# mikeoliphant/NeuralAudio

Measured on AMD Instinct MI355X. Metric: concurrent 48 kHz real-time streams + Msamples/s/GPU, NAM WaveNet Standard, higher is better.
Workload: dtype f32 (f16x3-split MFMA, f32 accumulate)

## Files before the change

neuralaudio_amd/csrc/wavenet_spec_impl.h:

```cpp
#pragma once

#include <algorithm>
#include <atomic>
#include <cstddef>
#include <cstdlib>

#include <hip/hip_runtime.h>

#include "device_once.h"
#include <cstring>
#include <type_traits>
#include <vector>

#include "tuning.h"
#include "wavenet_split_dev.h"

namespace na
{
	namespace spk
	{
		using namespace sp;

#ifndef NA_SPK_NT_DIL
#define NA_SPK_NT_DIL 256
#endif
#ifndef NA_SPK_NT_LD
#define NA_SPK_NT_LD 0
#endif
#ifndef NA_SPK_NT_ST
#define NA_SPK_NT_ST 0
#endif
#ifndef NA_SPK_DELAY
#define NA_SPK_DELAY 0
#endif
#ifndef NA_SPK_AUX2
#define NA_SPK_AUX2 0
#endif
		typedef __attribute__((address_space(3))) char* LdsPtr;
		__device__ __forceinline__ u32x4 LdsRead16(unsigned addr) { return *reinterpret_cast<__attribute__((address_space(3))) const u32x4*>((LdsPtr)(size_t)addr); }
		__device__ __forceinline__ u32x2 LdsRead8(unsigned addr) { return *reinterpret_cast<__attribute__((address_space(3))) const u32x2*>((LdsPtr)(size_t)addr); }
		__device__ __forceinline__ void LdsWrite16(unsigned addr, u32x4 v) { *reinterpret_cast<__attribute__((address_space(3))) u32x4*>((LdsPtr)(size_t)addr) = v; }

		template <bool COH>
		__device__ __forceinline__ float LoadIn(const float* p)
		{
			if constexpr (COH) return __builtin_bit_cast(float, __hip_atomic_load(reinterpret_cast<const unsigned*>(p), __ATOMIC_RELAXED, __HIP_MEMORY_SCOPE_SYSTEM));
			else return *p;
		}
		template <bool COH>
		__device__ __forceinline__ void StoreOut(float* p, float v)
		{
			if constexpr (COH) __hip_atomic_store(reinterpret_cast<unsigned*>(p), __builtin_bit_cast(unsigned, v), __ATOMIC_RELAXED, __HIP_MEMORY_SCOPE_SYSTEM);
			else *p = v;
		}

		struct ArchA1Base
		{
			static constexpr int K(int, int) { return 3; }
			static constexpr int HEADK = 1;
			static constexpr bool LEAKY = false;
			static constexpr int T = 2, CHUNK = 10;
			static constexpr bool COARSE = false;
			static constexpr bool GUARDHIST = false;
			static constexpr bool FOLD = false;
			static constexpr int SKEW = 0;
			static constexpr bool COMPACT = true;
#ifndef NA_A1_NT_DIL
#define NA_A1_NT_DIL 128
#endif
			static constexpr int NT_DIL = NA_A1_NT_DIL;
		};
#ifndef NA_SPK_SKEW
#define NA_SPK_SKEW 0
#endif
		struct ArchStd : ArchA1Base
		{
			static constexpr int SKEW = NA_SPK_SKEW;
			static constexpr bool FOLD = true;
			static constexpr int NA = 2;
			static constexpr int CH[2] = { 16, 8 };
			static constexpr int NLA[2] = { 10, 10 };
			static constexpr int DIL[2][16] = { { 1, 2, 4, 8, 16, 32, 64, 128, 256, 512 }, { 1, 2, 4, 8, 16, 32, 64, 128, 256, 512 } };
		};
		struct ArchLite : ArchA1Base
		{
			static constexpr int NA = 2;
			static constexpr int CH[2] = { 16, 8 };
			static constexpr int NLA[2] = { 7, 13 };
			static constexpr int DIL[2][16] = { { 1, 2, 4, 8, 16, 32, 64 }, { 128, 256, 512, 1, 2, 4, 8, 16, 32, 64, 128, 256, 512 } };
		};
		struct ArchLite16 : ArchA1Base
		{
			static constexpr int NA = 2;
			static constexpr int CH[2] = { 16, 16 };
			static constexpr int NLA[2] = { 7, 13 };
			static constexpr int DIL[2][16] = { { 1, 2, 4, 8, 16, 32, 64 }, { 128, 256, 512, 1, 2, 4, 8, 16, 32, 64, 128, 256, 512 } };
		};

		struct ArchLite16T1 : ArchLite16 { static constexpr int T = 1; };

		struct ArchA2Base
		{
			static constexpr int NA = 1;
			static constexpr int NLA[2] = { 23, 0 };
			static constexpr int DIL[2][32] = { { 1, 3, 7, 17, 41, 101, 239, 1, 3, 7, 17, 41, 101, 239, 1, 13, 1, 3, 7, 17, 41, 101, 239 }, { 0 } };
			static constexpr int K(int, int l) { return (l == 14 || l == 15) ? 15 : 6; }
			static constexpr int HEADK = 16;
			static constexpr bool LEAKY = true;
			static constexpr int CHUNK = 16;
			static constexpr bool COARSE = true;
			static constexpr bool GUARDHIST = true;
			static constexpr bool FOLD = false;
			static constexpr int SKEW = 0;
			static constexpr bool COMPACT = false;
			static constexpr int NT_DIL = 100;
		};
		struct ArchA2Full : ArchA2Base { static constexpr int CH[2] = { 8, 0 }; static constexpr int T = 2; };
		struct ArchA2Lite : ArchA2Base { static constexpr int CH[2] = { 4, 0 }; static constexpr int T = 4; };

		struct FamStd { typedef ArchStd A0; typedef ArchStd A1; static constexpr int N = 1; };
		struct FamLite { typedef ArchLite A0; typedef ArchLite A1; static constexpr int N = 1; };
		struct FamLitePacked { typedef ArchLite A0; typedef ArchLite16 A1; static constexpr int N = 2; };
		struct FamA2 { typedef ArchA2Full A0; typedef ArchA2Lite A1; static constexpr int N = 2; };
		struct FamLite16T1 { typedef ArchLite16T1 A0; typedef ArchLite16T1 A1; static constexpr int N = 1; };

		enum TapClass { TAP_LDS = 0, TAP_HIST = 1, TAP_BOTH = 2 };

		template <class A>
		struct Tab
		{
			static constexpr int NA = A::NA;
			static constexpr int TotalLayers() { int n = 0; for (int a = 0; a < NA; a++) n += A::NLA[a]; return n; }
			static constexpr int NL = TotalLayers();
			static constexpr int NSTAGES = NL + NA + 1;
			static constexpr int ArrOf(int L) { int a = 0; while (L >= A::NLA[a]) { L -= A::NLA[a]; a++; } return a; }
			static constexpr int InArr(int L) { int a = 0; while (L >= A::NLA[a]) { L -= A::NLA[a]; a++; } return L; }
			static constexpr int Dil(int L) { return A::DIL[ArrOf(L)][InArr(L)]; }
			static constexpr int GPof(int a) { return A::CH[a] / 4; }
			static constexpr bool FirstOfArr(int L) { return InArr(L) == 0; }
			static constexpr bool LastOfArr(int L) { return InArr(L) == A::NLA[ArrOf(L)] - 1; }
			static constexpr int KS(int L) { return A::K(ArrOf(L), InArr(L)); }
			static constexpr bool Fold(int L) { return A::FOLD && KS(L) == 3 && GPof(ArrOf(L)) >= 2; }
			static constexpr int HEADK = A::HEADK;
			static constexpr int NRINGS = NL + (HEADK > 1 ? 1 : 0);
			static constexpr bool ExactRing(int L) { return L < NL && !FirstOfArr(L) && Dil(L) >= FRAMES && (KS(L) - 1) * Dil(L) >= 2 * FRAMES && ((KS(L) - 1) * Dil(L)) % 16 == 0; }
			static constexpr int HistFrames(int L) { return L < NL ? ((KS(L) - 1) * Dil(L) + 15) / 16 * 16 : (HEADK - 1 + 15) / 16 * 16; }
			static constexpr bool CompactRing(int L) { return A::COMPACT && L < NL && KS(L) > 1 && HistFrames(L) <= WN_COMPACT_MAX_HISTORY; }
			static constexpr int RingFrames(int L)
			{
				if (ExactRing(L)) return (KS(L) - 1) * Dil(L);
				if (CompactRing(L)) return 3 * HistFrames(L);
				return HistFrames(L) + FRAMES;
			}
			static constexpr int RingKeep(int L) { return ExactRing(L) ? RingFrames(L) : (CompactRing(L) ? HistFrames(L) : RingFrames(L) - FRAMES); }
			static constexpr int RingG(int L) { return GPof(L < NL ? ArrOf(L) : NA - 1); }
			static constexpr int RingOff(int L)
			{
				int o = WN_HEADER_F4;
				for (int l = 0; l < L; l++) o += RingFrames(l) * RingG(l);
				return o;
			}
			static constexpr int StateF4 = (RingOff(NRINGS) + 15) / 16 * 16;
			static constexpr int StageOfLayer(int L) { return 1 + L + ArrOf(L); }
			static constexpr int FirstLayerOfArr(int a) { int L = 0; for (int i = 0; i < a; i++) L += A::NLA[i]; return L; }
			static constexpr int LinkStage(int a) { return FirstLayerOfArr(a) + a; }
			static constexpr int LinkNC(int a) { const int Po = 4 / GPof(a - 1), Pn = 4 / GPof(a); return Po > Pn ? Po : Pn; }
			static constexpr int LayerOfStage(int s)
			{
				for (int L = 0; L < NL; L++)
					if (StageOfLayer(L) == s) return L;
				return -1;
			}
			static constexpr int StageOps(int s)
			{
				if (s == 0) return 1;
				if (s == NSTAGES - 1) return 2 * HEADK + 1;
				for (int a = 1; a < NA; a++)
					if (s == LinkStage(a)) return 4 * LinkNC(a) + 1;
				return 2 * KS(LayerOfStage(s)) + 4;
			}
			static constexpr int AOff(int s) { int o = 0; for (int i = 0; i < s; i++) o += StageOps(i) * 64; return o; }
			static constexpr int WsplitQuads = AOff(NSTAGES);
			static constexpr int CHUNK = A::CHUNK;
			static constexpr int TapOps(int s) { return s == NSTAGES - 1 ? 2 * HEADK : 2 * KS(LayerOfStage(s)); }
			static constexpr bool Chunked(int s) { return StageOps(s) > CHUNK; }
			static constexpr int TapChunks(int s) { return (TapOps(s) + CHUNK - 1) / CHUNK; }
			static constexpr int NumChunks(int s) { return Chunked(s) ? TapChunks(s) + 1 : 1; }
			static constexpr int ChunkBegin(int s, int c)
			{
				if (!Chunked(s)) return 0;
				if (c >= TapChunks(s)) return TapOps(s);
				const int pairs = TapOps(s) / 2, n = TapChunks(s);
				return 2 * ((pairs * c + n - 1) / n);
			}
			static constexpr int ChunkEnd(int s, int c) { return !Chunked(s) ? StageOps(s) : (c >= TapChunks(s) ? StageOps(s) : ChunkBegin(s, c + 1)); }
			static constexpr int ChunkIndex(int s, int c) { int n = 0; for (int i = 0; i < s; i++) n += NumChunks(i); return n + c; }
			static constexpr int MaxChunkOps()
			{
				int m = 0;
				for (int s = 0; s < NSTAGES; s++)
					for (int c = 0; c < NumChunks(s); c++) m = (ChunkEnd(s, c) - ChunkBegin(s, c)) > m ? (ChunkEnd(s, c) - ChunkBegin(s, c)) : m;
				return m;
			}
			static constexpr int MaxGP() { int m = 0; for (int a = 0; a < NA; a++) m = GPof(a) > m ? GPof(a) : m; return m; }
		};

		template <class A_, int NF_, int SPB_, bool PK_, bool COH_ = false, bool NT_ = false>
		struct Cfg
		{
			static constexpr bool COH = COH_;
			static constexpr bool NT = NT_;
			typedef A_ A;
			typedef Tab<A_> TB;
			static constexpr int NF = NF_, T = A_::T, FW = 16 * T, WPS = NF_ / FW, SPB = SPB_ * T / 2, NTHREADS = 64 * WPS * SPB;
			static_assert(WPS >= 1 && WPS * FW == NF_, "block length is a whole number of waves");
			static constexpr bool PK = PK_;
			static constexpr int MAXOPS = A_::CHUNK;
			static_assert(TB::MaxChunkOps() <= MAXOPS, "stage operand chunk");
			static constexpr int HPF = 5;
			static constexpr int SKEW = (SPB == 2 && !PK_ && T == 2 && A_::SKEW > 0) ? A_::SKEW : 0;
			static constexpr int NWB = SKEW > 0 ? SPB : 1;
			static constexpr int STG_THREADS = NTHREADS / NWB;
			static constexpr bool AUX16 = !PK_ && SKEW == 0;
			static constexpr int AUX_OFF = 0;
			static constexpr int IMG_OFF = AUX_OFF + SPB * FRAMES * (PK_ ? 32 : (AUX16 ? 16 : 8));
			static constexpr int IMG_ONE = TB::MaxGP() * PLANE * 16;
			static constexpr int WBUF_OFF = IMG_OFF + SPB * 2 * IMG_ONE;
			static constexpr int WBUF_ONE = MAXOPS * 1024;
			static constexpr int IDOP_OFF = WBUF_OFF + NWB * 2 * WBUF_ONE;
			static constexpr int DUMP_OFF = IDOP_OFF + 1024;
			static constexpr int FLAG_OFF = DUMP_OFF + 1024;
			static constexpr int BCAST_OFF = FLAG_OFF + 16 * SPB;
			static constexpr int LDS_BYTES = BCAST_OFF + (COH_ ? 64 : 0);
			static_assert(LDS_BYTES <= 80 * 1024, "two workgroups per CU");
		};

		template <int GP, int T>
		struct Geo
		{
			static_assert(GP == 4 || GP == 2 || GP == 1, "full lane modes of 16 / 8 / 4 channels");
			static constexpr int P = 4 / GP;
			static_assert(T % P == 0, "every tile slot of a set is a tile of the wave");
			static constexpr int S = T / P;
		};

		constexpr int TapClassOf(int F0, int P, int i, int shift)
		{
			const int lo = F0 + 16 * P * i - shift, hi = lo + 16 * P - 1;
			return hi < 0 ? TAP_HIST : (lo >= 0 ? TAP_LDS : TAP_BOTH);
		}

		template <class C, int RG>
		constexpr bool SmallRing() { return C::A::GUARDHIST && C::TB::RingKeep(RG) <= GUARD; }

		template <class C>
		constexpr int WaveTapClass(int w, int P, int i, int shift, bool small)
		{
			if (small) return TAP_LDS;
			if (!C::A::COARSE || w == 0 || C::WPS <= 2) return TapClassOf(C::FW * w, P, i, shift);
			const int first = TapClassOf(C::FW * 1, P, i, shift);
			for (int v = 2; v < C::WPS; v++)
				if (TapClassOf(C::FW * v, P, i, shift) != first) return TAP_BOTH;
			return first;
		}

		template <class C, int L>
		struct LayerSig
		{
			typedef typename C::TB TB;
			static constexpr int GP = TB::GPof(TB::ArrOf(L)), P = Geo<GP, C::T>::P, S = Geo<GP, C::T>::S, d = TB::Dil(L), K = TB::KS(L);
			static constexpr bool NEXT = !TB::LastOfArr(L);
			static constexpr int LN = NEXT ? L + 1 : L;
			static constexpr int dn = NEXT ? TB::Dil(LN) : 0, Kn = NEXT ? TB::KS(LN) : 1;
			static constexpr bool FOLD = TB::Fold(L) && !C::PK;
			static constexpr unsigned long long Of(int w)
			{
				unsigned long long s = 0;
				for (int k = 0; k < K - 1; k++)
					for (int i = 0; i < S; i++) s = s * 3 + (unsigned)WaveTapClass<C>(w, P, i, d * (K - 1 - k), SmallRing<C, L>());
				for (int k = 0; k < Kn - 1 && k < C::HPF; k++)
					for (int i = 0; i < S; i++) s = s * 3 + (unsigned)WaveTapClass<C>(w, P, i, dn * (Kn - 1 - k), SmallRing<C, LN>());
				return s;
			}
			static constexpr int Rep(int w) { int r = w; for (int v = w - 1; v >= 0; v--) if (Of(v) == Of(w)) r = v; return r; }
			static constexpr unsigned MaskOf(int r) { unsigned m = 0; for (int w = 0; w < C::WPS; w++) if (Rep(w) == r) m |= 1u << w; return m; }
			static constexpr bool LastRep(int r) { for (int w = r + 1; w < C::WPS; w++) if (Rep(w) == w) return false; return true; }
		};

		struct Ctx
		{
			__amdgpu_buffer_rsrc_t srsrc;
			__amdgpu_buffer_rsrc_t wrsrc;
			int myPos;
			int wave, sub, waveAll;
			int lane;
			int gs0, gs1;
			unsigned wbuf;
			int stgWave;
#ifdef NA_SP_TRACE
			long long* trace;
			int nwaves;
#endif
		};

#ifdef NA_SP_TRACE
#define SPK_STAMP(stage, point) do { __builtin_amdgcn_sched_barrier(0); if (cx.trace != nullptr && cx.lane == 0) cx.trace[(((stage) * 8 + (point)) * cx.nwaves) + cx.waveAll] = (long long)__builtin_readcyclecounter(); __builtin_amdgcn_sched_barrier(0); } while (0)
#else
#define SPK_STAMP(stage, point) (void)0
#endif

		template <class C, int GP>
		struct Lanes
		{
			int fl;
			int cg;
			unsigned img;
			unsigned aux;
			unsigned ring;
			bool dual;

			__device__ __forceinline__ void Init(const Ctx& cx, int gs)
			{
				const int q = cx.lane >> 4, j = cx.lane & 15;
				const int p = q / GP;
				cg = q % GP;
				fl = 16 * p + j;
				const int f = C::FW * cx.wave + fl;
				img = (unsigned)(C::IMG_OFF + cx.sub * 2 * C::IMG_ONE + (cg * PLANE + GUARD + f) * 16);
				ring = (unsigned)((fl * GP + cg) * 16);
				dual = C::PK && gs < 0;
				if constexpr (C::PK) aux = (unsigned)(C::AUX_OFF + ((cx.sub * 4 + (gs < 0 ? 2 * cg : (cg >> gs))) * FRAMES + f) * 8);
				else aux = (unsigned)(C::AUX_OFF + (cx.sub * FRAMES + f) * (C::AUX16 ? 16 : 8));
			}
		};

		template <class C, int GP>
		__device__ __forceinline__ u32x4 AuxRead(const Lanes<C, GP>& ln, int i)
		{
			constexpr int P = Geo<GP, C::T>::P;
			if constexpr (C::AUX16) return LdsRead16(ln.aux + (unsigned)(16 * P * i * 16));
			else
			{
				const u32x2 v = LdsRead8(ln.aux + (unsigned)(16 * P * i * 8));
				if constexpr (C::PK)
				{
					if (ln.dual)
					{
						const u32x2 w = LdsRead8(ln.aux + (unsigned)(16 * P * i * 8) + (unsigned)(FRAMES * 8));
						return u32x4{ v.x, v.y, (v.x & 0xffffu) | (w.x << 16), (w.y & 0xffffu) | (w.x << 16) };
					}
				}
				return u32x4{ v.x, v.y, v.x & 0xffffu, 0u };
			}
		}

		struct State
		{
			f32x4 xc[2];
			f32x4 hd[2];
			u32x4 xs[2];
			u32x4 hist[5][2];
		};

		template <class C>
		__device__ __forceinline__ u32x4 Split(f32x4 v, const Ctx& cx)
		{
#ifdef NA_NO_SAT
			return SplitQuad(v);
#else
			if constexpr (C::A::LEAKY) return SplitQuadSat(v, (unsigned)(C::FLAG_OFF + 16 * cx.sub));
			else return SplitQuad(v);
#endif
		}

		template <int GP, int R>
		__device__ __forceinline__ int RingWrap(unsigned laneRing, int base)
		{
			unsigned a = laneRing + (unsigned)base * (unsigned)(GP * 16);
			return (int)__builtin_elementwise_min(a, a - (unsigned)(R * GP * 16));
		}

		template <class C, int RG, int WR>
		__device__ __forceinline__ u32x4 HistLoadAt(const Ctx& cx, unsigned laneRing, int fl, int shift, int i)
		{
			typedef typename C::TB TB;
			constexpr int GP = TB::RingG(RG), P = Geo<GP, C::T>::P, R = TB::RingFrames(RG), OFF = TB::RingOff(RG);
			const int cls = WaveTapClass<C>(WR, P, i, shift, SmallRing<C, RG>());
			if ((NA_ABL & 4) || cls == TAP_LDS) return RingLoad(cx.srsrc, OOB);
			const int pos0 = __builtin_amdgcn_readlane(cx.myPos, RG);
			int base = pos0 - shift + C::FW * cx.wave + 16 * P * i;
			if (base < 0) base += R;
			if (base >= R) base -= R;
			const int addr = RingWrap<GP, R>(laneRing, base);
			constexpr int NT_LD = C::NT ? 2 : NA_SPK_NT_LD, NT_DIL = C::NT ? C::A::NT_DIL : NA_SPK_NT_DIL;
			constexpr bool LONG = RG < TB::NL && TB::Dil(RG < TB::NL ? RG : 0) >= NT_DIL;
			if constexpr (LONG && NT_LD != 0)
			{
				if (cls == TAP_HIST) return RingLoadAux<NT_LD>(cx.srsrc, addr, OFF * 16);
				return RingLoadAux<NT_LD>(cx.srsrc, (C::FW * cx.wave + 16 * P * i + fl < shift) ? addr : OOB, OFF * 16);
			}
			if (cls == TAP_HIST) return RingLoad(cx.srsrc, addr, OFF * 16);
			return RingLoad(cx.srsrc, (C::FW * cx.wave + 16 * P * i + fl < shift) ? addr : OOB, OFF * 16);
		}

		template <class C, int L>
		constexpr int ShiftOf(int k) { return C::TB::Dil(L) * (C::TB::KS(L) - 1 - k); }

		template <class C, int GP>
		constexpr bool HistNeededAt(int shift, int i, bool small) { return !small && TapClassOf(0, Geo<GP, C::T>::P, i, shift) != TAP_LDS; }

		template <class C, int L>
		constexpr int PrefetchTaps() { return (C::TB::KS(L) - 1) < C::HPF ? (C::TB::KS(L) - 1) : C::HPF; }
		template <class C, int L>
		constexpr int HistLoadsOf()
		{
			typedef typename C::TB TB;
			constexpr int GP = TB::GPof(TB::ArrOf(L)), S = Geo<GP, C::T>::S;
			int n = 0;
			for (int k = 0; k < PrefetchTaps<C, L>(); k++)
				for (int i = 0; i < S; i++) n += HistNeededAt<C, GP>(ShiftOf<C, L>(k), i, SmallRing<C, L>()) ? 1 : 0;
			return n;
		}

		template <class C, int L, int WR>
		__device__ __forceinline__ void HistPrefetch(const Ctx& cx, unsigned laneRing, int fl, State& st)
		{
			constexpr int GP = C::TB::GPof(C::TB::ArrOf(L)), S = Geo<GP, C::T>::S;
#pragma unroll
			for (int k = 0; k < PrefetchTaps<C, L>(); k++)
#pragma unroll
				for (int i = 0; i < S; i++)
					if (HistNeededAt<C, GP>(ShiftOf<C, L>(k), i, SmallRing<C, L>())) st.hist[k][i] = HistLoadAt<C, L, WR>(cx, laneRing, fl, ShiftOf<C, L>(k), i);
		}

		template <class C, int RG>
		constexpr bool StoreNeeded(int i)
		{
			typedef typename C::TB TB;
			constexpr int P = Geo<TB::RingG(RG), C::T>::P, KEEP = TB::RingKeep(RG);
			return (C::NF - C::FW) + 16 * P * (i + 1) - 1 >= C::NF - KEEP;
		}
		template <class C, int RG>
		constexpr int StoresOf()
		{
			constexpr int S = Geo<C::TB::RingG(RG), C::T>::S;
			int n = 0;
			for (int i = 0; i < S; i++) n += StoreNeeded<C, RG>(i) ? 1 : 0;
			return n;
		}

		template <class C, int RG, int GP, int MINSHIFT>
		__device__ __forceinline__ void Publish(const Ctx& cx, const Lanes<C, GP>& ln, u32x4 v, int i, int imgWrite)
		{
			typedef typename C::TB TB;
			constexpr int P = Geo<GP, C::T>::P, R = TB::RingFrames(RG), OFF = TB::RingOff(RG), KEEP = TB::RingKeep(RG);
			static_assert(GP == TB::RingG(RG), "lane mode of the receiving ring");
			if (!(NA_ABL & 64) && MINSHIFT < C::NF)
				LdsWrite16(ln.img + (unsigned)(imgWrite * C::IMG_ONE + 16 * P * i * 16), v);
			if ((NA_ABL & 4) || !StoreNeeded<C, RG>(i)) return;
			const int pos0 = __builtin_amdgcn_readlane(cx.myPos, RG);
			int base;
			if constexpr (TB::CompactRing(RG))
			{
				int end = pos0 + C::NF % R;
				if (end >= R) end -= R;
				base = end - C::NF + C::FW * cx.wave + 16 * P * i + R;
			}
			else
			{
				base = pos0 + C::FW * cx.wave + 16 * P * i;
				if (base >= R) base -= R;
			}
			const int addr = RingWrap<GP, R>(ln.ring, base);
			constexpr int NT_ST = C::NT ? 2 : NA_SPK_NT_ST, NT_DIL = C::NT ? C::A::NT_DIL : NA_SPK_NT_DIL;
			constexpr bool LONG = RG < TB::NL && TB::Dil(RG < TB::NL ? RG : 0) >= NT_DIL;
			if constexpr (LONG && NT_ST != 0)
			{
				if (KEEP >= C::NF) RingStoreAux<NT_ST>(cx.srsrc, v, addr, OFF * 16);
				else RingStoreAux<NT_ST>(cx.srsrc, v, (C::FW * cx.wave + 16 * P * i + ln.fl >= C::NF - KEEP) ? addr : OOB, OFF * 16);
				return;
			}
			if (KEEP >= C::NF) RingStore(cx.srsrc, v, addr, OFF * 16);
			else RingStore(cx.srsrc, v, (C::FW * cx.wave + 16 * P * i + ln.fl >= C::NF - KEEP) ? addr : OOB, OFF * 16);
		}

		template <class C, int RG, int GP>
		__device__ __forceinline__ void GuardStage(const Ctx& cx, const Lanes<C, GP>& ln, int imgBuf)
		{
			typedef typename C::TB TB;
			static_assert(GP == TB::RingG(RG), "lane mode of the ring");
			constexpr int R = TB::RingFrames(RG), OFF = TB::RingOff(RG);
			if constexpr (!C::A::GUARDHIST) return;
			if (cx.wave != 0) return;
			if constexpr (SmallRing<C, RG>())
			{
				if (NA_ABL & 4) return;
				const int pos0 = __builtin_amdgcn_readlane(cx.myPos, RG);
				int base = pos0 - GUARD;
				if (base < 0) base += R;
				if (cx.lane < 16)
				{
#pragma unroll
					for (int cg = 0; cg < GP; cg++)
					{
						const int addr = RingWrap<GP, R>((unsigned)((cx.lane * GP + cg) * 16), base);
						const unsigned dst = (unsigned)(C::IMG_OFF + imgBuf * C::IMG_ONE + cg * PLANE * 16) + (unsigned)(cx.sub * 2 * C::IMG_ONE);
						__builtin_amdgcn_raw_ptr_buffer_load_lds(cx.srsrc, (__attribute__((address_space(3))) void*)(LdsPtr)(size_t)dst, 16, addr, OFF * 16, 0, 0);
					}
				}
			}
			else
			{
				if ((cx.lane >> 4) < GP && (cx.lane & 15) == 15) LdsWrite16(ln.img + (unsigned)(imgBuf * C::IMG_ONE) - 16u * 16u, u32x4{ 0, 0, 0, 0 });
			}
		}

		template <class C, int SN, int CN>
		struct Stager
		{
			typedef typename C::TB TB;
			static constexpr int QUADS = (TB::ChunkEnd(SN, CN) - TB::ChunkBegin(SN, CN)) * 64;
			static constexpr int SRC = TB::AOff(SN) + TB::ChunkBegin(SN, CN) * 64;
			static constexpr int BUF = TB::ChunkIndex(SN, CN) & 1;
			static constexpr int NCOPY = (QUADS + C::STG_THREADS - 1) / C::STG_THREADS;
			static __device__ __forceinline__ void Begin(const Ctx& cx)
			{
				if (NA_ABL & 16) return;
#pragma unroll
				for (int c = 0; c < NCOPY; c++)
				{
					const int i0 = c * C::STG_THREADS + cx.stgWave * 64;
					const bool mine = i0 < QUADS;
					const unsigned dst = mine ? cx.wbuf + (unsigned)(BUF * C::WBUF_ONE) + (unsigned)i0 * 16u : (unsigned)C::DUMP_OFF;
					__builtin_amdgcn_raw_ptr_buffer_load_lds(cx.wrsrc, (__attribute__((address_space(3))) void*)(LdsPtr)(size_t)dst, 16,
						mine ? (SRC + i0 + cx.lane) * 16 : OOB, 0, 0, 0);
				}
			}
			template <int LATER>
			static __device__ __forceinline__ void End()
			{
				__builtin_amdgcn_s_waitcnt((LATER & 15) | ((LATER >> 4) << 14) | (7 << 4) | (15 << 8));
			}
		};
		template <class C, int s, int c>
		struct NextChunk
		{
			static constexpr bool SAME = c + 1 < C::TB::NumChunks(s);
			static constexpr int S = SAME ? s : s + 1, CN = SAME ? c + 1 : 0;
			typedef Stager<C, S, CN> St;
		};

		template <class C>
		__device__ __forceinline__ u32x4 WOp(const Ctx& cx, int s, int c, int m)
		{
			const int buf = C::TB::ChunkIndex(s, c) & 1, local = m - C::TB::ChunkBegin(s, c);
			return LdsRead16(cx.wbuf + (unsigned)(buf * C::WBUF_ONE + ((NA_ABL & 128) ? 0 : local) * 1024) + (unsigned)cx.lane * 16u);
		}

		template <bool PACKED>
		__device__ __forceinline__ f32x4 ActivateTanh(f32x4 a)
		{
			if (PACKED)
			{
				const f32x2 lo = FastTanh2(f32x2{ a.x, a.y }), hi = FastTanh2(f32x2{ a.z, a.w });
				return f32x4{ lo.x, lo.y, hi.x, hi.y };
			}
			return f32x4{ FastTanh(a.x), FastTanh(a.y), FastTanh(a.z), FastTanh(a.w) };
		}

		template <class C, int GP>
		__device__ __forceinline__ u32x4 TapLds(const Ctx& cx, const Lanes<C, GP>& ln, int imgRead, int shift, int i, int cls)
		{
			constexpr int P = Geo<GP, C::T>::P;
			if (NA_ABL & 256) return u32x4{ (unsigned)shift, 0, 0, 0 };
			if (cls == TAP_LDS) return LdsRead16(ln.img + (unsigned)(imgRead * C::IMG_ONE) + (unsigned)((16 * P * i - shift) * 16));
			int off = C::FW * cx.wave + 16 * P * i + ln.fl - shift;
			off = off < -1 ? -1 : off;
			return LdsRead16((unsigned)(C::IMG_OFF + imgRead * C::IMG_ONE + GUARD * 16) + (unsigned)(cx.sub * 2 * C::IMG_ONE) + (unsigned)((ln.cg * PLANE + off) * 16));
		}

		template <class C, int RG, int GP, int WR>
		__device__ __forceinline__ f32x4 ConvTap(const Ctx& cx, const Lanes<C, GP>& ln, int imgRead, int shift, int i, u32x4 ah, u32x4 al, u32x4 hist, f32x4 acc)
		{
			constexpr int P = Geo<GP, C::T>::P;
			const int cls = WaveTapClass<C>(WR, P, i, shift, SmallRing<C, RG>());
			if (cls != TAP_LDS)
			{
				acc = Mfma(ah, hist, acc);
				acc = MfmaLo<1>(al, hist, acc);
			}
			if (cls != TAP_HIST)
			{
				const u32x4 b = TapLds<C, GP>(cx, ln, imgRead, shift, i, cls);
				acc = Mfma(ah, b, acc);
				acc = MfmaLo<1>(al, b, acc);
			}
			return acc;
		}

		template <class C, int RG, int GP, int WR>
		__device__ __forceinline__ f32x4 ConvTapFold(const Ctx& cx, const Lanes<C, GP>& ln, int imgRead, int shift, int i, u32x4 ah, u32x4 hist, f32x4 acc, u32x2& th)
		{
			constexpr int P = Geo<GP, C::T>::P;
			const int cls = WaveTapClass<C>(WR, P, i, shift, SmallRing<C, RG>());
			th = u32x2{ 0, 0 };
			if (cls != TAP_LDS)
			{
				acc = Mfma(ah, hist, acc);
				th = u32x2{ hist.x, hist.y };
			}
			if (cls != TAP_HIST)
			{
				const u32x4 b = TapLds<C, GP>(cx, ln, imgRead, shift, i, cls);
				acc = Mfma(ah, b, acc);
				th = cls == TAP_LDS ? u32x2{ b.x, b.y } : u32x2{ th.x | b.x, th.y | b.y };
			}
			return acc;
		}

		template <class C, int L, int WR, int c>
		__device__ __forceinline__ void LayerChunk(const Ctx& cx, const Lanes<C, C::TB::GPof(C::TB::ArrOf(L))>& ln, State& st, u32x4 (&ax)[LayerSig<C, L>::S],
			f32x4 (&acc)[LayerSig<C, L>::S])
		{
			typedef typename C::TB TB;
			typedef LayerSig<C, L> SG;
			constexpr int GP = SG::GP, S = SG::S, K = SG::K, s = TB::StageOfLayer(L), NCH = TB::NumChunks(s), CB = TB::ChunkBegin(s, c), CE = TB::ChunkEnd(s, c);
			constexpr int imgRead = s & 1, imgWrite = (s + 1) & 1, LN = SG::LN;
			constexpr bool LASTLAYER = TB::LastOfArr(L) && TB::ArrOf(L) == TB::NA - 1;
			constexpr int NEXTMINSHIFT = SG::NEXT ? TB::Dil(LN) : (1 << 20);
			constexpr bool OWN = 2 * (K - 1) >= CB && 2 * (K - 1) < CE;
			constexpr bool TAIL = 2 * K >= CB && 2 * K < CE;
			constexpr int LATER = ((OWN && SG::NEXT) ? HistLoadsOf<C, LN>() : 0) + ((TAIL && SG::NEXT && !LASTLAYER) ? StoresOf<C, LN>() : 0);
			typedef typename NextChunk<C, s, c>::St NextStager;
			if constexpr (c == 0)
			{
				if constexpr (SG::NEXT) GuardStage<C, LN, GP>(cx, ln, imgWrite);
				else if constexpr (LASTLAYER && TB::HEADK > 1) GuardStage<C, TB::NL, GP>(cx, ln, (TB::NSTAGES - 1 + 1) & 1);
			}
			NextStager::Begin(cx);
			if constexpr (c == 0)
			{
#pragma unroll
				for (int i = 0; i < S; i++) ax[i] = AuxRead<C, GP>(ln, i);
			}
			constexpr int KLO = CB / 2, KHI = (CE / 2 < K - 1) ? CE / 2 : K - 1;
			constexpr int NX = (KHI > C::HPF) ? KHI - (KLO > C::HPF ? KLO : C::HPF) : 0;
			u32x4 hx[NX > 0 ? NX : 1][S];
#pragma unroll
			for (int k = KLO; k < KHI; k++)
			{
				if (k < C::HPF) continue;
#pragma unroll
				for (int i = 0; i < S; i++)
					if (WaveTapClass<C>(WR, SG::P, i, ShiftOf<C, L>(k), SmallRing<C, L>()) != TAP_LDS) hx[k - (KLO > C::HPF ? KLO : C::HPF)][i] = HistLoadAt<C, L, WR>(cx, ln.ring, ln.fl, ShiftOf<C, L>(k), i);
			}
			static_assert(!SG::FOLD || (NCH == 1 && K == 3), "folded operands: K = 3 layers in one chunk");
			u32x2 th[SG::FOLD ? 2 : 1][S];
#pragma unroll
			for (int k = KLO; k < KHI; k++)
			{
				const u32x4 ah = WOp<C>(cx, s, c, 2 * k), al = SG::FOLD ? ah : WOp<C>(cx, s, c, 2 * k + 1);
#pragma unroll
				for (int i = 0; i < S; i++)
				{
					u32x4 h = u32x4{ 0, 0, 0, 0 };
					if (WaveTapClass<C>(WR, SG::P, i, ShiftOf<C, L>(k), SmallRing<C, L>()) != TAP_LDS)
						h = (k < C::HPF) ? st.hist[k < C::HPF ? k : 0][i] : hx[k >= C::HPF ? k - (KLO > C::HPF ? KLO : C::HPF) : 0][i];
					if constexpr (SG::FOLD) acc[i] = ConvTapFold<C, L, GP, WR>(cx, ln, imgRead, ShiftOf<C, L>(k), i, ah, h, acc[i], th[k < 2 ? k : 0][i]);
					else acc[i] = ConvTap<C, L, GP, WR>(cx, ln, imgRead, ShiftOf<C, L>(k), i, ah, al, h, acc[i]);
				}
			}
			if constexpr (SG::FOLD)
			{
				const u32x4 al01 = WOp<C>(cx, s, c, 1);
#pragma unroll
				for (int i = 0; i < S; i++) acc[i] = Mfma(al01, u32x4{ th[0][i].x, th[0][i].y, th[1][i].x, th[1][i].y }, acc[i]);
			}
			if constexpr (OWN)
			{
				if constexpr (SG::NEXT) HistPrefetch<C, LN, WR>(cx, ln.ring, ln.fl, st);
				const u32x4 ah = WOp<C>(cx, s, c, 2 * K - 2), al = WOp<C>(cx, s, c, 2 * K - 1);
#pragma unroll
				for (int i = 0; i < S; i++)
				{
					acc[i] = Mfma(ah, st.xs[i], acc[i]);
					if constexpr (SG::FOLD) acc[i] = Mfma(al, u32x4{ st.xs[i].x, st.xs[i].y, ax[i].x, ax[i].y }, acc[i]);
					else acc[i] = MfmaLo<1>(al, st.xs[i], acc[i]);
				}
			}
			if constexpr (TAIL)
			{
				if constexpr (!SG::FOLD)
				{
					const u32x4 xa = WOp<C>(cx, s, c, 2 * K);
#pragma unroll
					for (int i = 0; i < S; i++) acc[i] = Mfma(xa, ax[i], acc[i]);
				}
				SPK_STAMP(s, 1);
				f32x4 z[S];
#pragma unroll
				for (int i = 0; i < S; i++)
				{
					if constexpr (C::A::LEAKY) z[i] = f32x4{ LeakyReLU(acc[i].x), LeakyReLU(acc[i].y), LeakyReLU(acc[i].z), LeakyReLU(acc[i].w) };
					else z[i] = ActivateTanh<(NA_PK_TANH != 0) && (C::NTHREADS < 512)>(acc[i]);
				}
				SPK_STAMP(s, 2);
				const u32x4 idop = LdsRead16((unsigned)C::IDOP_OFF + (unsigned)cx.lane * 16u);
				const u32x4 w1h = WOp<C>(cx, s, c, 2 * K + 1), w1l = WOp<C>(cx, s, c, 2 * K + 2), b1a = SG::FOLD ? w1l : WOp<C>(cx, s, c, 2 * K + 3);
#pragma unroll
				for (int i = 0; i < S; i++)
				{
					const u32x4 zs = SplitQuad(z[i]);
					st.hd[i] = Mfma(idop, zs, st.hd[i]);
					if constexpr (!LASTLAYER)
					{
						f32x4 y = st.xc[i];
						y = Mfma(w1h, zs, y);
						const u32x4 axi = NA_SPK_AUX2 ? AuxRead<C, GP>(ln, i) : ax[i];
						if constexpr (SG::FOLD) y = Mfma(w1l, u32x4{ zs.x, zs.y, axi.x, axi.y }, y);
						else
						{
							y = MfmaLo<2>(w1l, zs, y);
							y = Mfma(b1a, axi, y);
						}
						st.xc[i] = y;
						if constexpr (SG::NEXT)
						{
							st.xs[i] = Split<C>(y, cx);
							Publish<C, LN, GP, NEXTMINSHIFT>(cx, ln, st.xs[i], i, imgWrite);
						}
					}
				}
				SPK_STAMP(s, 3);
			}
			NextStager::template End<LATER>();
			SPK_STAMP(s, 4);
			BlockBarrier<C::NTHREADS / 64>();
			if constexpr (c + 1 < NCH) LayerChunk<C, L, WR, c + 1>(cx, ln, st, ax, acc);
		}

		template <class C, int L, int WR>
		__device__ __forceinline__ void LayerBody(const Ctx& cx, const Lanes<C, C::TB::GPof(C::TB::ArrOf(L))>& ln, State& st)
		{
			constexpr int S = LayerSig<C, L>::S;
			SPK_STAMP(C::TB::StageOfLayer(L), 0);
			u32x4 ax[S];
			f32x4 acc[S];
#pragma unroll
			for (int i = 0; i < S; i++) acc[i] = f32x4{ 0.0f, 0.0f, 0.0f, 0.0f };
			LayerChunk<C, L, WR, 0>(cx, ln, st, ax, acc);
			SPK_STAMP(C::TB::StageOfLayer(L), 5);
		}

		template <class C, int L, int W>
		__device__ __forceinline__ void LayerDispatch(const Ctx& cx, const Lanes<C, C::TB::GPof(C::TB::ArrOf(L))>& ln, State& st)
		{
			typedef LayerSig<C, L> SG;
			if constexpr (W < C::WPS)
			{
				if constexpr (SG::Rep(W) != W) LayerDispatch<C, L, W + 1>(cx, ln, st);
				else if constexpr (SG::LastRep(W)) LayerBody<C, L, W>(cx, ln, st);
				else
				{
					constexpr unsigned MASK = SG::MaskOf(W);
					if ((MASK >> cx.wave) & 1u) LayerBody<C, L, W>(cx, ln, st);
					else LayerDispatch<C, L, W + 1>(cx, ln, st);
				}
			}
		}

		template <class C, int L, int W>
		__device__ __forceinline__ void FirstHistDispatch(const Ctx& cx, unsigned laneRing, int fl, State& st)
		{
			typedef typename C::TB TB;
			constexpr int GP = TB::GPof(TB::ArrOf(L)), P = Geo<GP, C::T>::P, S = Geo<GP, C::T>::S;
			if constexpr (W < C::WPS)
			{
				constexpr bool same = [] {
					bool r = true;
					for (int w = W + 1; w < C::WPS; w++)
						for (int k = 0; k < PrefetchTaps<C, L>(); k++)
							for (int i = 0; i < S; i++) r = r && WaveTapClass<C>(w, P, i, ShiftOf<C, L>(k), SmallRing<C, L>()) == WaveTapClass<C>(W, P, i, ShiftOf<C, L>(k), SmallRing<C, L>());
					return r;
				}();
				if constexpr (same) HistPrefetch<C, L, W>(cx, laneRing, fl, st);
				else
				{
					if (cx.wave == W) HistPrefetch<C, L, W>(cx, laneRing, fl, st);
					else FirstHistDispatch<C, L, W + 1>(cx, laneRing, fl, st);
				}
			}
		}

		template <class C>
		__device__ __forceinline__ void RechStage(const Ctx& cx, const Lanes<C, C::TB::GPof(0)>& ln, State& st)
		{
			constexpr int GP = C::TB::GPof(0), S = Geo<GP, C::T>::S;
			SPK_STAMP(0, 0);
			GuardStage<C, 0, GP>(cx, ln, 1);
			const u32x4 ra = WOp<C>(cx, 0, 0, 0);
#pragma unroll
			for (int i = 0; i < S; i++)
			{
				const u32x4 ax = AuxRead<C, GP>(ln, i);
				f32x4 x = f32x4{ 0.0f, 0.0f, 0.0f, 0.0f };
				x = Mfma(ra, ax, x);
				st.xc[i] = x;
				st.hd[i] = f32x4{ 0.0f, 0.0f, 0.0f, 0.0f };
				st.xs[i] = Split<C>(x, cx);
				Publish<C, 0, GP, C::TB::Dil(0)>(cx, ln, st.xs[i], i, 1);
			}
			FirstHistDispatch<C, 0, 0>(cx, ln.ring, ln.fl, st);
			SPK_STAMP(0, 1); SPK_STAMP(0, 2); SPK_STAMP(0, 3);
			Stager<C, 1, 0>::template End<StoresOf<C, 0>() + HistLoadsOf<C, 0>()>();
			SPK_STAMP(0, 4);
			BlockBarrier<C::NTHREADS / 64>();
			SPK_STAMP(0, 5);
		}

		template <class C, int AN>
		__device__ __forceinline__ void LinkStage(const Ctx& cx, const Lanes<C, C::TB::GPof(AN)>& ln, State& st)
		{
			typedef typename C::TB TB;
			constexpr int GPO = TB::GPof(AN - 1), GPN = TB::GPof(AN), Po = 4 / GPO, Pn = 4 / GPN, NC = Po > Pn ? Po : Pn;
			constexpr int So = Geo<GPO, C::T>::S, Sn = Geo<GPN, C::T>::S, s = TB::LinkStage(AN), LN = TB::FirstLayerOfArr(AN);
			static_assert(C::T == 1 || C::T == 2, "array links are written for one or two tiles per wave");
			SPK_STAMP(s, 0);
			GuardStage<C, LN, GPN>(cx, ln, (s + 1) & 1);
			Stager<C, s + 1, 0>::Begin(cx);
			u32x4 hs[So], xq[So];
#pragma unroll
			for (int i = 0; i < So; i++)
			{
				hs[i] = Split<C>(st.hd[i], cx);
				xq[i] = Split<C>(st.xc[i], cx);
			}
			f32x4 hn[Sn], xn[Sn];
#pragma unroll
			for (int i = 0; i < Sn; i++)
			{
				hn[i] = f32x4{ 0.0f, 0.0f, 0.0f, 0.0f };
				xn[i] = f32x4{ 0.0f, 0.0f, 0.0f, 0.0f };
				hn[i] = Mfma(WOp<C>(cx, s, 0, 4 * NC), AuxRead<C, GPN>(ln, i), hn[i]);
			}
#pragma unroll
			for (int t = 0; t < C::T; t++)
			{
				const int u = t % NC, so = t / Po, sn = t / Pn;
hn[sn] = Mfma(WOp<C>(cx, s, 0, 4 * u), hs[so], hn[sn]);
				hn[sn] = MfmaLo<4>(WOp<C>(cx, s, 0, 4 * u + 1), hs[so], hn[sn]);
				xn[sn] = Mfma(WOp<C>(cx, s, 0, 4 * u + 2), xq[so], xn[sn]);
				xn[sn] = MfmaLo<4>(WOp<C>(cx, s, 0, 4 * u + 3), xq[so], xn[sn]);
			}
#pragma unroll
			for (int i = 0; i < Sn; i++)
			{
				st.hd[i] = hn[i];
				st.xc[i] = xn[i];
				st.xs[i] = Split<C>(xn[i], cx);
				Publish<C, LN, GPN, TB::Dil(LN)>(cx, ln, st.xs[i], i, (s + 1) & 1);
			}
			FirstHistDispatch<C, LN, 0>(cx, ln.ring, ln.fl, st);
			SPK_STAMP(s, 1); SPK_STAMP(s, 2); SPK_STAMP(s, 3);
			Stager<C, s + 1, 0>::template End<StoresOf<C, LN>() + HistLoadsOf<C, LN>()>();
			SPK_STAMP(s, 4);
			BlockBarrier<C::NTHREADS / 64>();
			SPK_STAMP(s, 5);
		}

		template <class C, int WR>
		__device__ __forceinline__ void HeadBody(const Ctx& cx, const Lanes<C, C::TB::GPof(C::TB::NA - 1)>& ln, State& st, float* __restrict__ out, size_t outBase,
			const long (&outRow)[4], int pack, float headScale, bool live)
		{
			typedef typename C::TB TB;
			constexpr int GP = TB::GPof(TB::NA - 1), P = Geo<GP, C::T>::P, S = Geo<GP, C::T>::S, s = TB::NSTAGES - 1, K = TB::HEADK, NCH = TB::NumChunks(s), RG = TB::NL;
			constexpr int imgHead = (s + 1) & 1;
			u32x4 hs[S];
			f32x4 acc[S];
#pragma unroll
			for (int i = 0; i < S; i++)
			{
				hs[i] = Split<C>(st.hd[i], cx);
				acc[i] = f32x4{ 0.0f, 0.0f, 0.0f, 0.0f };
			}
#pragma unroll
			for (int c = 0; c < NCH; c++)
			{
				if constexpr (K > 1)
				{
					if (c + 1 < NCH)
					{
						if (c == 0) Stager<C, s, 1>::Begin(cx);
						else if (c + 1 < NCH) Stager<C, s, (NCH > 2 ? 2 : 1)>::Begin(cx);
					}
					if (c == 0)
					{
#pragma unroll
						for (int i = 0; i < S; i++) Publish<C, RG, GP, 1>(cx, ln, hs[i], i, imgHead);
						BlockBarrier<C::NTHREADS / 64>();
					}
#pragma unroll
					for (int k = 0; k < K - 1; k++)
					{
						if (2 * k < TB::ChunkBegin(s, c) || 2 * k >= TB::ChunkEnd(s, c)) continue;
						const u32x4 ah = WOp<C>(cx, s, c, 2 * k), al = WOp<C>(cx, s, c, 2 * k + 1);
#pragma unroll
						for (int i = 0; i < S; i++)
						{
							u32x4 h = u32x4{ 0, 0, 0, 0 };
							if (WaveTapClass<C>(WR, P, i, K - 1 - k, SmallRing<C, RG>()) != TAP_LDS) h = HistLoadAt<C, RG, WR>(cx, ln.ring, ln.fl, K - 1 - k, i);
							acc[i] = ConvTap<C, RG, GP, WR>(cx, ln, imgHead, K - 1 - k, i, ah, al, h, acc[i]);
						}
					}
				}
				if (2 * (K - 1) >= TB::ChunkBegin(s, c) && 2 * (K - 1) < TB::ChunkEnd(s, c))
				{
					const u32x4 ah = WOp<C>(cx, s, c, 2 * K - 2), al = WOp<C>(cx, s, c, 2 * K - 1);
#pragma unroll
					for (int i = 0; i < S; i++)
					{
						acc[i] = Mfma(ah, hs[i], acc[i]);
						acc[i] = MfmaLo<8>(al, hs[i], acc[i]);
					}
				}
				if (2 * K >= TB::ChunkBegin(s, c) && 2 * K < TB::ChunkEnd(s, c))
				{
					const u32x4 ba = WOp<C>(cx, s, c, 2 * K);
#pragma unroll
					for (int i = 0; i < S; i++)
					{
						acc[i] = Mfma(ba, AuxRead<C, GP>(ln, i), acc[i]);
						const int f = C::FW * cx.wave + 16 * P * i + ln.fl;
						if (live && ln.cg == 0)
						{
							if constexpr (C::PK)
							{
								const float v[4] = { acc[i].x, acc[i].y, acc[i].z, acc[i].w };
#pragma unroll
								for (int q = 0; q < 4; q++)
									if (q < pack && outRow[q] >= 0) StoreOut<C::COH>(out + outRow[q] + f, headScale * v[q]);
							}
							else StoreOut<C::COH>(out + outBase + f, headScale * acc[i].x);
						}
					}
				}
				if (c + 1 < NCH)
				{
					__builtin_amdgcn_s_waitcnt(0 | (7 << 4) | (15 << 8));
					BlockBarrier<C::NTHREADS / 64>();
				}
			}
		}

		template <class C>
		__device__ __forceinline__ void HeadDispatch(const Ctx& cx, const Lanes<C, C::TB::GPof(C::TB::NA - 1)>& ln, State& st, float* __restrict__ out, size_t outBase,
			const long (&outRow)[4], int pack, float headScale, bool live)
		{
			if constexpr (C::TB::HEADK == 1 || C::WPS == 1 || SmallRing<C, C::TB::NL>()) HeadBody<C, 0>(cx, ln, st, out, outBase, outRow, pack, headScale, live);
			else
			{
				if (cx.wave == 0) HeadBody<C, 0>(cx, ln, st, out, outBase, outRow, pack, headScale, live);
				else HeadBody<C, C::WPS - 1>(cx, ln, st, out, outBase, outRow, pack, headScale, live);
			}
		}

		template <class C, int L, int LEND>
		__device__ __forceinline__ void RunLayers(const Ctx& cx, const Lanes<C, C::TB::GPof(C::TB::ArrOf(L))>& ln, State& st)
		{
			LayerDispatch<C, L, 0>(cx, ln, st);
			if constexpr (L + 1 < LEND) RunLayers<C, L + 1, LEND>(cx, ln, st);
		}

		template <class C, int AN>
		__device__ __forceinline__ void RunArrays(const Ctx& cx, State& st, float* __restrict__ out, size_t outBase, const long (&outRow)[4], int pack, float headScale, bool live)
		{
			typedef typename C::TB TB;
			Lanes<C, TB::GPof(AN)> ln;
			ln.Init(cx, AN == 0 ? cx.gs0 : cx.gs1);
			if constexpr (AN == 0) RechStage<C>(cx, ln, st);
			else LinkStage<C, AN>(cx, ln, st);
			RunLayers<C, TB::FirstLayerOfArr(AN), TB::FirstLayerOfArr(AN) + C::A::NLA[AN]>(cx, ln, st);
			if constexpr (AN + 1 < TB::NA) RunArrays<C, AN + 1>(cx, st, out, outBase, outRow, pack, headScale, live);
			else HeadDispatch<C>(cx, ln, st, out, outBase, outRow, pack, headScale, live);
		}

		template <class C>
		__device__ __forceinline__ void RunWorkgroup(const GroupArgs& ga, int groupBlock, const float* __restrict__ in, float* __restrict__ out, long inStride, long outStride
#ifdef NA_SP_TRACE
			, long long* trace
#endif
			, const int tid = (int)threadIdx.x
			)
		{
			typedef typename C::TB TB;
			constexpr bool PK = C::PK;
			constexpr int SPB = C::SPB, NF = C::NF;
			const int lane = tid & 63;
			const int waveAll = __builtin_amdgcn_readfirstlane(tid >> 6);
			const int sub = waveAll / C::WPS, wave = waveAll % C::WPS;

			int sidx = groupBlock * SPB + sub;
			const bool live = sidx < ga.numStreams;
			if (!live) sidx = ga.numStreams - 1;
			const int slot = ga.slots ? ga.slots[sidx] : ga.slot0 + sidx;
			const int row = PK ? 0 : (ga.slots ? ga.rows[sidx] : ga.row0 + sidx);
			u32x4* stt = ga.state + (size_t)slot * (size_t)ga.stateF4;
			int* header = reinterpret_cast<int*>(stt);

			Ctx cx;
			cx.srsrc = MakeRsrc(stt, live ? (unsigned)ga.stateF4 * 16u : 0u);
			cx.wrsrc = MakeRsrc(ga.wsplit, (unsigned)ga.wsplitQuads * 16u);
			cx.myPos = header[lane];
			cx.wave = wave; cx.sub = sub; cx.waveAll = waveAll; cx.lane = lane;
			cx.wbuf = (unsigned)(C::WBUF_OFF + (C::SKEW > 0 ? sub : 0) * 2 * C::WBUF_ONE);
			cx.stgWave = C::SKEW > 0 ? wave : waveAll;
#ifdef NA_SP_TRACE
			cx.trace = trace;
// ... 513 lines not shown
```

Before: 3691.

## Add lean mode: per-wave ring stores/hist loads, live-only weight staging, fused BOTH taps

Adds a LEAN mode, enabled by default for the Standard architecture, with three parts. Ring stores and history loads are issued only by the waves whose frames actually need them, and wait counts become per-wave. Weight staging copies only the live operand slots of folded K=3 layers. Taps that straddle history and LDS are merged with a bitwise OR so they need one MFMA instead of two. The aim is fewer global memory ops, less staging traffic and fewer MFMAs per layer. The cost is more template dispatch per wave and a reliance on the zero-fill assumption that makes the OR merge correct.

```diff
diff --git a/neuralaudio_amd/csrc/wavenet_spec_impl.h b/neuralaudio_amd/csrc/wavenet_spec_impl.h
--- a/neuralaudio_amd/csrc/wavenet_spec_impl.h
+++ b/neuralaudio_amd/csrc/wavenet_spec_impl.h
@@ -32,6 +32,9 @@
 #endif
 #ifndef NA_SPK_DELAY
 #define NA_SPK_DELAY 0
+#endif
+#ifndef NA_SPK_LEAN
+#define NA_SPK_LEAN 6
 #endif
 #ifndef NA_SPK_AUX2
 #define NA_SPK_AUX2 0
@@ -69,6 +72,7 @@
 #define NA_A1_NT_DIL 128
 #endif
 			static constexpr int NT_DIL = NA_A1_NT_DIL;
+			static constexpr bool LEAN = false;
 		};
 #ifndef NA_SPK_SKEW
 #define NA_SPK_SKEW 0
@@ -77,6 +81,7 @@
 		{
 			static constexpr int SKEW = NA_SPK_SKEW;
 			static constexpr bool FOLD = true;
+			static constexpr bool LEAN = true;
 			static constexpr int NA = 2;
 			static constexpr int CH[2] = { 16, 8 };
 			static constexpr int NLA[2] = { 10, 10 };
@@ -114,6 +119,7 @@
 			static constexpr int SKEW = 0;
 			static constexpr bool COMPACT = false;
 			static constexpr int NT_DIL = 100;
+			static constexpr bool LEAN = false;
 		};
 		struct ArchA2Full : ArchA2Base { static constexpr int CH[2] = { 8, 0 }; static constexpr int T = 2; };
 		struct ArchA2Lite : ArchA2Base { static constexpr int CH[2] = { 4, 0 }; static constexpr int T = 4; };
@@ -221,6 +227,8 @@
 			static constexpr int SKEW = (SPB == 2 && !PK_ && T == 2 && A_::SKEW > 0) ? A_::SKEW : 0;
 			static constexpr int NWB = SKEW > 0 ? SPB : 1;
 			static constexpr int STG_THREADS = NTHREADS / NWB;
+			static constexpr bool LEAN = A_::LEAN && !PK_ && !COH_ && SKEW == 0 && T == 2;
+			static constexpr bool LEAN_MEM = LEAN && (NA_SPK_LEAN & 1), LEAN_STAGE = LEAN && (NA_SPK_LEAN & 2), LEAN_MFMA = LEAN && (NA_SPK_LEAN & 4);
 			static constexpr bool AUX16 = !PK_ && SKEW == 0;
 			static constexpr int AUX_OFF = 0;
 			static constexpr int IMG_OFF = AUX_OFF + SPB * FRAMES * (PK_ ? 32 : (AUX16 ? 16 : 8));
@@ -264,6 +272,14 @@
 			return first;
 		}
 
+		template <class C, int RG>
+		constexpr bool StoreMine(int w, int i)
+		{
+			typedef typename C::TB TB;
+			constexpr int P = Geo<TB::RingG(RG), C::T>::P, KEEP = TB::RingKeep(RG);
+			return C::FW * w + 16 * P * (i + 1) - 1 >= C::NF - KEEP;
+		}
+
 		template <class C, int L>
 		struct LayerSig
 		{
@@ -280,6 +296,8 @@
 					for (int i = 0; i < S; i++) s = s * 3 + (unsigned)WaveTapClass<C>(w, P, i, d * (K - 1 - k), SmallRing<C, L>());
 				for (int k = 0; k < Kn - 1 && k < C::HPF; k++)
 					for (int i = 0; i < S; i++) s = s * 3 + (unsigned)WaveTapClass<C>(w, P, i, dn * (Kn - 1 - k), SmallRing<C, LN>());
+				if constexpr (C::LEAN_MEM && NEXT)
+					for (int i = 0; i < S; i++) s = s * 2 + (StoreMine<C, LN>(w, i) ? 1u : 0u);
 				return s;
 			}
 			static constexpr int Rep(int w) { int r = w; for (int v = w - 1; v >= 0; v--) if (Of(v) == Of(w)) r = v; return r; }
@@ -411,14 +429,22 @@
 
 		template <class C, int L>
 		constexpr int PrefetchTaps() { return (C::TB::KS(L) - 1) < C::HPF ? (C::TB::KS(L) - 1) : C::HPF; }
+
 		template <class C, int L>
-		constexpr int HistLoadsOf()
+		constexpr bool HistIssuedBy(int w, int k, int i)
 		{
 			typedef typename C::TB TB;
-			constexpr int GP = TB::GPof(TB::ArrOf(L)), S = Geo<GP, C::T>::S;
+			constexpr int GP = TB::GPof(TB::ArrOf(L)), P = Geo<GP, C::T>::P;
+			if (!HistNeededAt<C, GP>(ShiftOf<C, L>(k), i, SmallRing<C, L>())) return false;
+			return !C::LEAN_MEM || WaveTapClass<C>(w, P, i, ShiftOf<C, L>(k), SmallRing<C, L>()) != TAP_LDS;
+		}
+		template <class C, int L>
+		constexpr int HistLoadsOfWave(int w)
+		{
+			constexpr int S = Geo<C::TB::GPof(C::TB::ArrOf(L)), C::T>::S;
 			int n = 0;
 			for (int k = 0; k < PrefetchTaps<C, L>(); k++)
-				for (int i = 0; i < S; i++) n += HistNeededAt<C, GP>(ShiftOf<C, L>(k), i, SmallRing<C, L>()) ? 1 : 0;
+				for (int i = 0; i < S; i++) n += HistIssuedBy<C, L>(w, k, i) ? 1 : 0;
 			return n;
 		}
 
@@ -430,7 +456,7 @@
 			for (int k = 0; k < PrefetchTaps<C, L>(); k++)
 #pragma unroll
 				for (int i = 0; i < S; i++)
-					if (HistNeededAt<C, GP>(ShiftOf<C, L>(k), i, SmallRing<C, L>())) st.hist[k][i] = HistLoadAt<C, L, WR>(cx, laneRing, fl, ShiftOf<C, L>(k), i);
+					if (HistIssuedBy<C, L>(WR, k, i)) st.hist[k][i] = HistLoadAt<C, L, WR>(cx, laneRing, fl, ShiftOf<C, L>(k), i);
 		}
 
 		template <class C, int RG>
@@ -441,15 +467,15 @@
 			return (C::NF - C::FW) + 16 * P * (i + 1) - 1 >= C::NF - KEEP;
 		}
 		template <class C, int RG>
-		constexpr int StoresOf()
+		constexpr int StoresOfWave(int w)
 		{
 			constexpr int S = Geo<C::TB::RingG(RG), C::T>::S;
 			int n = 0;
-			for (int i = 0; i < S; i++) n += StoreNeeded<C, RG>(i) ? 1 : 0;
+			for (int i = 0; i < S; i++) n += (StoreNeeded<C, RG>(i) && (!C::LEAN_MEM || StoreMine<C, RG>(w, i))) ? 1 : 0;
 			return n;
 		}
 
-		template <class C, int RG, int GP, int MINSHIFT>
+		template <class C, int RG, int GP, int MINSHIFT, int WR = -1>
 		__device__ __forceinline__ void Publish(const Ctx& cx, const Lanes<C, GP>& ln, u32x4 v, int i, int imgWrite)
 		{
 			typedef typename C::TB TB;
@@ -458,6 +484,10 @@
 			if (!(NA_ABL & 64) && MINSHIFT < C::NF)
 				LdsWrite16(ln.img + (unsigned)(imgWrite * C::IMG_ONE + 16 * P * i * 16), v);
 			if ((NA_ABL & 4) || !StoreNeeded<C, RG>(i)) return;
+			if constexpr (C::LEAN_MEM)
+			{
+				if (WR >= 0 ? !StoreMine<C, RG>(WR, i) : (C::FW * cx.wave + 16 * P * (i + 1) - 1 < C::NF - KEEP)) return;
+			}
 			const int pos0 = __builtin_amdgcn_readlane(cx.myPos, RG);
 			int base;
 			if constexpr (TB::CompactRing(RG))
@@ -523,9 +553,29 @@
 			static constexpr int SRC = TB::AOff(SN) + TB::ChunkBegin(SN, CN) * 64;
 			static constexpr int BUF = TB::ChunkIndex(SN, CN) & 1;
 			static constexpr int NCOPY = (QUADS + C::STG_THREADS - 1) / C::STG_THREADS;
+			static constexpr int LSN = TB::LayerOfStage(SN) < 0 ? 0 : TB::LayerOfStage(SN);
+			static constexpr bool LIVEONLY = C::LEAN_STAGE && TB::LayerOfStage(SN) >= 0 && TB::Fold(LSN) && !TB::Chunked(SN);
+			static constexpr int NLIVE = (TB::LastOfArr(LSN) && TB::ArrOf(LSN) == TB::NA - 1) ? 5 : 7;
+			static constexpr int STG_WAVES = C::STG_THREADS / 64;
+			static constexpr int NCOPY_LIVE = (NLIVE + STG_WAVES - 1) / STG_WAVES;
 			static __device__ __forceinline__ void Begin(const Ctx& cx)
 			{
 				if (NA_ABL & 16) return;
+				if constexpr (LIVEONLY)
+				{
+					static_assert(TB::StageOps(SN) == 10 && CN == 0, "operands of a folded K = 3 layer");
+#pragma unroll
+					for (int c = 0; c < NCOPY_LIVE; c++)
+					{
+						const int j = c * STG_WAVES + cx.stgWave;
+						const bool mine = j < NLIVE;
+						const int op = j + (j > 2 ? 1 : 0) + (j > 4 ? 1 : 0);
+						const unsigned dst = mine ? cx.wbuf + (unsigned)(BUF * C::WBUF_ONE) + (unsigned)op * 1024u : (unsigned)C::DUMP_OFF;
+						__builtin_amdgcn_raw_ptr_buffer_load_lds(cx.wrsrc, (__attribute__((address_space(3))) void*)(LdsPtr)(size_t)dst, 16,
+							mine ? (SRC + op * 64 + cx.lane) * 16 : OOB, 0, 0, 0);
+					}
+					return;
+				}
 #pragma unroll
 				for (int c = 0; c < NCOPY; c++)
 				{
@@ -604,6 +654,13 @@
 			constexpr int P = Geo<GP, C::T>::P;
 			const int cls = WaveTapClass<C>(WR, P, i, shift, SmallRing<C, RG>());
 			th = u32x2{ 0, 0 };
+			if (C::LEAN_MFMA && cls == TAP_BOTH)
+			{
+				const u32x4 b = TapLds<C, GP>(cx, ln, imgRead, shift, i, cls);
+				acc = Mfma(ah, u32x4{ hist.x | b.x, hist.y | b.y, hist.z | b.z, hist.w | b.w }, acc);
+				th = u32x2{ hist.x | b.x, hist.y | b.y };
+				return acc;
+			}
 			if (cls != TAP_LDS)
 			{
 				acc = Mfma(ah, hist, acc);
@@ -630,7 +687,7 @@
 			constexpr int NEXTMINSHIFT = SG::NEXT ? TB::Dil(LN) : (1 << 20);
 			constexpr bool OWN = 2 * (K - 1) >= CB && 2 * (K - 1) < CE;
 			constexpr bool TAIL = 2 * K >= CB && 2 * K < CE;
-			constexpr int LATER = ((OWN && SG::NEXT) ? HistLoadsOf<C, LN>() : 0) + ((TAIL && SG::NEXT && !LASTLAYER) ? StoresOf<C, LN>() : 0);
+			constexpr int LATER = ((OWN && SG::NEXT) ? HistLoadsOfWave<C, LN>(WR) : 0) + ((TAIL && SG::NEXT && !LASTLAYER) ? StoresOfWave<C, LN>(WR) : 0);
 			typedef typename NextChunk<C, s, c>::St NextStager;
 			if constexpr (c == 0)
 			{
@@ -727,7 +784,7 @@
 						if constexpr (SG::NEXT)
 						{
 							st.xs[i] = Split<C>(y, cx);
-							Publish<C, LN, GP, NEXTMINSHIFT>(cx, ln, st.xs[i], i, imgWrite);
+							Publish<C, LN, GP, NEXTMINSHIFT, WR>(cx, ln, st.xs[i], i, imgWrite);
 						}
 					}
 				}
@@ -792,6 +849,23 @@
 			}
 		}
 
+		template <class C, class St, int L, int W>
+		__device__ __forceinline__ void EndFirst(const Ctx& cx)
+		{
+			constexpr int N = StoresOfWave<C, L>(W) + HistLoadsOfWave<C, L>(W);
+			constexpr bool same = [] {
+				bool r = true;
+				for (int w = W + 1; w < C::WPS; w++) r = r && StoresOfWave<C, L>(w) + HistLoadsOfWave<C, L>(w) == N;
+				return r;
+			}();
+			if constexpr (same) St::template End<N>();
+			else
+			{
+				if (cx.wave == W) St::template End<N>();
+				else EndFirst<C, St, L, W + 1>(cx);
+			}
+		}
+
 		template <class C>
 		__device__ __forceinline__ void RechStage(const Ctx& cx, const Lanes<C, C::TB::GPof(0)>& ln, State& st)
 		{
@@ -812,7 +886,7 @@
 			}
 			FirstHistDispatch<C, 0, 0>(cx, ln.ring, ln.fl, st);
 			SPK_STAMP(0, 1); SPK_STAMP(0, 2); SPK_STAMP(0, 3);
-			Stager<C, 1, 0>::template End<StoresOf<C, 0>() + HistLoadsOf<C, 0>()>();
+			EndFirst<C, Stager<C, 1, 0>, 0, 0>(cx);
 			SPK_STAMP(0, 4);
 			BlockBarrier<C::NTHREADS / 64>();
 			SPK_STAMP(0, 5);
@@ -862,7 +936,7 @@
 			}
 			FirstHistDispatch<C, LN, 0>(cx, ln.ring, ln.fl, st);
 			SPK_STAMP(s, 1); SPK_STAMP(s, 2); SPK_STAMP(s, 3);
-			Stager<C, s + 1, 0>::template End<StoresOf<C, LN>() + HistLoadsOf<C, LN>()>();
+			EndFirst<C, Stager<C, s + 1, 0>, LN, 0>(cx);
 			SPK_STAMP(s, 4);
 			BlockBarrier<C::NTHREADS / 64>();
 			SPK_STAMP(s, 5);
```

After: 3810 (median of 6 runs). 3.2% higher.
